# Yiming-M/CLIP-EBC

Hardware: AMD Instinct MI355X
Metric: train crops/sec clip_vit_b_16 224px @1/2/4/8 MI355X; MAE parity (higher is better)
Workload: dtype fp16; 1 GPU; clip_vit_b_16 224x224 deep-VPT(32) + DACE/DMCount train step, 16 crops/GPU, AMP fp16, NWPU anchors (BASELINE configs[2]); global_batch=16, seq_len=229, parallelism=dp1

## Files before the change

### clip-ebc_amd/csrc/attention.hip

```cpp
#include <algorithm>
#include <cstdlib>
#include <string>

#include "ebc_common.h"
#include "kernels.h"
#include "mfma.h"
#include "touch.h"

using namespace ebc;

#ifndef EBC_ATTN_STAMP
#define EBC_ATTN_STAMP(phase) ((void)0)
#endif

namespace {

constexpr int HD = 64;
constexpr int LP = 256;
constexpr int NKT = LP / 16;
constexpr float LOG2E = 1.4426950408889634f;
__device__ __forceinline__ int attn_block() { return xcd_remap(blockIdx.x, (int)gridDim.x); }

template <class E> struct AttnCfg {
    using T = typename E::T;
// ... 364 lines not shown
#pragma unroll
            for (int dt = 0; dt < HD / 16; ++dt) row[16 * dt + fr] = E::from(dq_acc[dt][i] * scale);
        }
    }
}

template <class E, int NWV, int LFIX>
__global__ __launch_bounds__(64 * NWV) void attn_bwd_dq_kernel(const typename E::T* __restrict__ qkv, const typename E::T* __restrict__ dout,
                                                          const typename E::T* __restrict__ out, const float* __restrict__ lse,
                                                          float* __restrict__ delta, typename E::T* __restrict__ dqkv, int B,
                                                          int L_, int H, float scale)
{
    attn_bwd_dq_body<E, NWV, LFIX>(attn_block(), qkv, dout, out, lse, delta, dqkv, B, L_, H, scale);
}

template <class E>
__device__ __forceinline__ float attn_delta_row(const typename E::T* drow, const typename E::T* orow) {
    float p[4];
#pragma unroll
    for (int fg = 0; fg < 4; ++fg) {
        float dd = 0.f;
#pragma unroll
        for (int ks = 0; ks < 2; ++ks) {
            const typename E::Frag df = load8<E>(drow + 32 * ks + 8 * fg), of = load8<E>(orow + 32 * ks + 8 * fg);
#pragma unroll
            for (int j = 0; j < 8; ++j) dd = fmaf((float)df[j], (float)of[j], dd);
        }
        p[fg] = dd;
    }
    return (p[0] + p[1]) + (p[2] + p[3]);
}

template <class E>
__device__ __forceinline__ float attn_delta_quad(const typename E::T* drow, const typename E::T* orow) {
    const typename E::Frag d0 = load8<E>(drow), d1 = load8<E>(drow + 8), o0 = load8<E>(orow), o1 = load8<E>(orow + 8);
    float acc = 0.f;
#pragma unroll
    for (int j = 0; j < 8; j += 2) {
        if constexpr (std::is_same<E, EF16>::value) {
            typedef _Float16 h2 __attribute__((ext_vector_type(2)));
            acc = __builtin_amdgcn_fdot2(h2{d0[j], d0[j + 1]}, h2{o0[j], o0[j + 1]}, acc, false);
            acc = __builtin_amdgcn_fdot2(h2{d1[j], d1[j + 1]}, h2{o1[j], o1[j + 1]}, acc, false);
        } else {
            typedef __bf16 b2 __attribute__((ext_vector_type(2)));
            acc = __builtin_amdgcn_fdot2_f32_bf16(b2{d0[j], d0[j + 1]}, b2{o0[j], o0[j + 1]}, acc, false);
            acc = __builtin_amdgcn_fdot2_f32_bf16(b2{d1[j], d1[j + 1]}, b2{o1[j], o1[j + 1]}, acc, false);
        }
    }
    acc += __builtin_amdgcn_update_dpp(0.f, acc, 0xB1, 0xF, 0xF, false);
    acc += __builtin_amdgcn_update_dpp(0.f, acc, 0x4E, 0xF, 0xF, false);
    return acc;
}

template <class E, int NWV, int LFIX>
__device__ __forceinline__ void attn_bwd_dkv_body(int bid, const typename E::T* __restrict__ qkv, const typename E::T* __restrict__ dout,
                                                  const typename E::T* __restrict__ out, const float* __restrict__ lse,
                                                  const float* __restrict__ delta, typename E::T* __restrict__ dqkv, int B,
                                                  int L_, int H, float scale)
{
    const int L = LFIX > 0 ? LFIX : L_;
    using T = typename E::T;
    using C = AttnCfg<E>;
    extern __shared__ __attribute__((aligned(16))) char smem[];
    T* Qs = reinterpret_cast<T*>(smem);
    T* Ds = reinterpret_cast<T*>(smem + C::TILE_BYTES);
    float* ls = reinterpret_cast<float*>(smem + 2 * C::TILE_BYTES);
    float* dl = ls + LP;
    constexpr int QB = 16 * NWV;
    const int nkb = (L + QB - 1) / QB;
    const int bh = bid / nkb, kb = bid % nkb;
    const int b = bh / H, h = bh % H;
    const int D3 = 3 * H * HD, D = H * HD;
    const T* base = qkv + (size_t)b * L * D3 + h * HD;
    RowFetch<E, NWV> fq, fd;
    rows_fetch<E, NWV>(fq, base, D3, L);
    rows_fetch<E, NWV>(fd, dout + (size_t)b * L * D + h * HD, D, L);
    const int lane = threadIdx.x & 63, w = threadIdx.x >> 6, fr = lane & 15, fg = lane >> 4;
    const int k0 = kb * QB + w * 16;
    const int kme = k0 + fr;
    const bool kv = kme < L;
    typename E::Frag kf[2], vf[2];
#pragma unroll
    for (int ks = 0; ks < 2; ++ks) {
        kf[ks] = gload8<E>(base + (size_t)kme * D3 + D + 32 * ks + 8 * fg, kv);
// ... 64 lines not shown
                                                           const float* __restrict__ lse, const float* __restrict__ delta,
                                                           typename E::T* __restrict__ dqkv, int B, int L_, int H, float scale)
{
    attn_bwd_dkv_body<E, NWV, LFIX>(attn_block(), qkv, dout, nullptr, lse, delta, dqkv, B, L_, H, scale);
}

struct AttnLaneOffsets {
    int row[2];
    int col[HD / 16];
    __device__ __forceinline__ AttnLaneOffsets() {
        const int l = threadIdx.x & 63, fr = l & 15, fg = l >> 4;
        const int sr = attn_swz(fr);
#pragma unroll
        for (int ks = 0; ks < 2; ++ks) row[ks] = (fr * HD + (((4 * ks + fg) ^ sr) << 3)) * 2;
        const int g = l >> 4, w = l & 15, q = w >> 2, p = w & 3, rr = 4 * g + q, sc = attn_swz(rr);
#pragma unroll
        for (int dt = 0; dt < HD / 16; ++dt) col[dt] = (rr * HD + ((((2 * dt + (p >> 1)) ^ sc) << 3) | (4 * (p & 1)))) * 2;
    }
};
template <class E>
__device__ __forceinline__ typename E::Frag rowfrag_at(const char* tile, int off, int t) {
    return __builtin_bit_cast(typename E::Frag, *reinterpret_cast<const uint4*>(tile + off + t * 16 * HD * 2));
}
template <class E>
__device__ __forceinline__ typename E::Frag colfrag_at(const char* tile, int off, int st) {
    const char* a = tile + off + st * 32 * HD * 2;
    const s16x4 lo = __builtin_amdgcn_ds_read_tr16_b64_v4i16((__attribute__((address_space(3))) s16x4*)(a));
    const s16x4 hi = __builtin_amdgcn_ds_read_tr16_b64_v4i16((__attribute__((address_space(3))) s16x4*)(a + 16 * HD * 2));
    typedef short s16x8 __attribute__((ext_vector_type(8)));
    s16x8 v = {lo[0], lo[1], lo[2], lo[3], hi[0], hi[1], hi[2], hi[3]};
    return __builtin_bit_cast(typename E::Frag, v);
}

template <class E, int LFIX>
__global__ __launch_bounds__(1024) void attn_bwd_one_kernel(const typename E::T* __restrict__ qkv, const typename E::T* __restrict__ dout,
                                                           const typename E::T* __restrict__ out, const float* __restrict__ lse,
                                                           typename E::T* __restrict__ dqkv, int B, int L_, int H, float scale,
                                                           int rows, TouchList touch)
{
    constexpr int NWV = 16;
    const int L = LFIX > 0 ? LFIX : L_;
    using T = typename E::T;
    using C = AttnCfg<E>;
    EBC_ATTN_STAMP(0);
    extern __shared__ __attribute__((aligned(16))) char smem[];
    T* Ks = reinterpret_cast<T*>(smem);
    T* Vs = reinterpret_cast<T*>(smem + C::TILE_BYTES);
    T* Qs = reinterpret_cast<T*>(smem + 2 * C::TILE_BYTES);
    T* Ds = reinterpret_cast<T*>(smem + 3 * C::TILE_BYTES);
    float* ls = reinterpret_cast<float*>(smem + 4 * C::TILE_BYTES);
    float* dl = ls + LP;
    const int bh = attn_block(), b = bh / H, h = bh % H;
    const int D3 = 3 * H * HD, D = H * HD;
    const T* base = qkv + (size_t)b * L * D3 + h * HD;
    const T* dob = dout + (size_t)b * L * D + h * HD;
    RowFetch<E, NWV> fk, fv, fq, fd;
    rows_fetch<E, NWV>(fk, base + D, D3, L);
    rows_fetch<E, NWV>(fv, base + 2 * D, D3, L);
    rows_fetch<E, NWV>(fq, base, D3, L);
    rows_fetch<E, NWV>(fd, dob, D, L);
    const int qd = threadIdx.x >> 2, qj = threadIdx.x & 3;
    float lsv = INFINITY, dlv = 0.f;
    if (qd < L) {
        if (qj == 0) lsv = lse[((size_t)b * H + h) * L + qd] * LOG2E;
        dlv = attn_delta_quad<E>(dob + (size_t)qd * D + 16 * qj, out + ((size_t)b * L + qd) * D + h * HD + 16 * qj);
    }
    rows_store<E, NWV>(Ks, fk);
    rows_store<E, NWV>(Vs, fv);
    rows_store<E, NWV>(Qs, fq);
    rows_store<E, NWV>(Ds, fd);
    static_assert(64 * NWV >= 4 * LP, "a lane quad per padded query");
    if (qj == 0) { ls[qd] = lsv; dl[qd] = dlv; }
    __syncthreads();
    EBC_ATTN_STAMP(1);

    const int lane = threadIdx.x & 63, w = threadIdx.x >> 6, fr = lane & 15, fg = lane >> 4;
    const int lim = rows > 0 && rows < L ? rows : L;
    TouchSink tsink;
    if (touch.n) touch_issue<NWV>(touch, tsink);
    if (16 * w >= lim) {
        if (touch.n) touch_wait(tsink);
        EBC_ATTN_STAMP(2);
        return;
    }
    const int nkt = (L + 15) >> 4;
    const bool ragged = (L & 15) != 0;
    const float c2 = scale * LOG2E;
    static_assert(E::BYTES == 2, "swizzled 16-bit tiles");
    const AttnLaneOffsets lo;
    const char* Kr[2] = {reinterpret_cast<const char*>(Ks) + lo.row[0], reinterpret_cast<const char*>(Ks) + lo.row[1]};
    const char* Vr[2] = {reinterpret_cast<const char*>(Vs) + lo.row[0], reinterpret_cast<const char*>(Vs) + lo.row[1]};
    const char* Qr[2] = {reinterpret_cast<const char*>(Qs) + lo.row[0], reinterpret_cast<const char*>(Qs) + lo.row[1]};
    const char* Dr[2] = {reinterpret_cast<const char*>(Ds) + lo.row[0], reinterpret_cast<const char*>(Ds) + lo.row[1]};
    const char* Kc[HD / 16];
    const char* Qc[HD / 16];
    const char* Dc[HD / 16];
#pragma unroll
    for (int dt = 0; dt < HD / 16; ++dt) {
        Kc[dt] = reinterpret_cast<const char*>(Ks) + lo.col[dt];
        Qc[dt] = reinterpret_cast<const char*>(Qs) + lo.col[dt];
        Dc[dt] = reinterpret_cast<const char*>(Ds) + lo.col[dt];
    }
    {
        const int q0 = 16 * w, qme = q0 + fr;
        typename E::Frag qf[2], df[2];
// ... 510 lines not shown
    return EBC_OK;
}
template <class E> int attn_fwd_t(const void* qkv, void* out, float* lse, int B, int L, int H, hipStream_t st,
                                  const TouchList* touch)
{
    if (attn_fwd_waves(B, L, H) == 16)
        return L == L_VPT32 ? attn_fwd_nw<E, 16, L_VPT32>(qkv, out, lse, B, L, H, st, touch)
                            : attn_fwd_nw<E, 16, 0>(qkv, out, lse, B, L, H, st, touch);
    return L == L_VPT32 ? attn_fwd_nw<E, 8, L_VPT32>(qkv, out, lse, B, L, H, st, touch)
                        : attn_fwd_nw<E, 8, 0>(qkv, out, lse, B, L, H, st, touch);
}

template <class E, int NW, int LFIX> int attn_bwd_nw(const void* qkv, const void* dout, const void* out, const float* lse,
                                                     float* delta, void* dqkv, int B, int L, int H, hipStream_t st)
{
    using C = AttnCfg<E>;
    const size_t lds_dq = 2 * C::TILE_BYTES, lds_kv = 2 * C::TILE_BYTES + 2 * LP * sizeof(float);
    if (!ensure_lds<attn_bwd_dq_kernel<E, NW, LFIX>>((int)lds_dq, st) || !ensure_lds<attn_bwd_dkv_kernel<E, NW, LFIX>>((int)lds_kv, st))
        return EBC_E_LAUNCH;
    const int grid = B * H * ((L + 16 * NW - 1) / (16 * NW));
    int pi = probe_on() ? probe_start(EBC_PROBE_ATTN_BWD_DQ, 0, 0, 0, 0, B, L, H, st) : -1;
    hipLaunchKernelGGL((attn_bwd_dq_kernel<E, NW, LFIX>), dim3(grid), dim3(64 * NW), lds_dq, st, (const typename E::T*)qkv,
                       (const typename E::T*)dout, (const typename E::T*)out, lse, delta, (typename E::T*)dqkv, B, L, H,
                       0.125f);
    probe_stop(pi, st);
    EBC_CHECK_LAUNCH();
    pi = probe_on() ? probe_start(EBC_PROBE_ATTN_BWD_DKV, 0, 0, 0, 0, B, L, H, st) : -1;
    hipLaunchKernelGGL((attn_bwd_dkv_kernel<E, NW, LFIX>), dim3(grid), dim3(64 * NW), lds_kv, st, (const typename E::T*)qkv,
                       (const typename E::T*)dout, lse, delta, (typename E::T*)dqkv, B, L, H, 0.125f);
    probe_stop(pi, st);
    EBC_CHECK_LAUNCH();
    return EBC_OK;
}
template <class E, int LFIX> int attn_bwd_one(const void* qkv, const void* dout, const void* out, const float* lse,
                                              void* dqkv, int B, int L, int H, hipStream_t st, int rows, const TouchList* touch)
{
    using C = AttnCfg<E>;
    const size_t lds = 4 * C::TILE_BYTES + 2 * LP * sizeof(float);
    if (!ensure_lds<attn_bwd_one_kernel<E, LFIX>>((int)lds, st)) return EBC_E_LAUNCH;
    const TouchList t = touch && g_touch_mode == 1 ? *touch : TouchList{};
    const int pi = probe_on() ? probe_start(EBC_PROBE_ATTN_BWD_DQ, 1, 0, 0, 0, B, L, H, st) : -1;
    hipLaunchKernelGGL((attn_bwd_one_kernel<E, LFIX>), dim3(B * H), dim3(1024), lds, st, (const typename E::T*)qkv,
                       (const typename E::T*)dout, (const typename E::T*)out, lse, (typename E::T*)dqkv, B, L, H, 0.125f,
                       rows, t);
    probe_stop(pi, st);
    EBC_CHECK_LAUNCH();
    return EBC_OK;
}


template <class E> int attn_bwd_t(const void* qkv, const void* dout, const void* out, const float* lse, float* delta,
                                  void* dqkv, int B, int L, int H, hipStream_t st, int rows, const TouchList* touch)
{
    if constexpr (E::BYTES == 2) {
        return L == L_VPT32 ? attn_bwd_one<E, L_VPT32>(qkv, dout, out, lse, dqkv, B, L, H, st, rows, touch)
                            : attn_bwd_one<E, 0>(qkv, dout, out, lse, dqkv, B, L, H, st, rows, touch);
    }
    if (attn_waves(L) == 16)
        return L == L_VPT32 ? attn_bwd_nw<E, 16, L_VPT32>(qkv, dout, out, lse, delta, dqkv, B, L, H, st)
                            : attn_bwd_nw<E, 16, 0>(qkv, dout, out, lse, delta, dqkv, B, L, H, st);
    return attn_bwd_nw<E, 8, 0>(qkv, dout, out, lse, delta, dqkv, B, L, H, st);
}

}

namespace ebc {
bool touch_enabled() { return g_touch_mode == 1; }
}

extern "C" int ebc_set_weight_touch(int mode)
{
    if (mode < 0 || mode > 1) return EBC_E_ARG;
    g_touch_mode = mode;
    return EBC_OK;
}

namespace ebc {
// ... 6 lines not shown
            case EBC_F32: return attn_fwd_long<EF32>(qkv, out, lse, B, L, H, st);
            case EBC_F16: return attn_fwd_long<EF16>(qkv, out, lse, B, L, H, st);
            case EBC_BF16: return attn_fwd_long<EBF16>(qkv, out, lse, B, L, H, st);
        }
        return EBC_E_ARG;
    }
    switch (dtype) {
        case EBC_F32: return attn_fwd_t<EF32>(qkv, out, lse, B, L, H, st, nullptr);
        case EBC_F16: return attn_fwd_t<EF16>(qkv, out, lse, B, L, H, st, touch);
        case EBC_BF16: return attn_fwd_t<EBF16>(qkv, out, lse, B, L, H, st, touch);
    }
    return EBC_E_ARG;
}
int attention_bwd(int dtype, const void* qkv, const void* dout, const void* out, const float* lse, float* delta,
                  void* dqkv, int B, int L, int H, hipStream_t st, int rows, const TouchList* touch)
{
    if (L <= 0 || L > L_MAX || B <= 0 || H <= 0 || rows < 0) return EBC_E_UNSUPPORTED;
    if (L > LP) {
        if (!delta || !lse) return EBC_E_ARG;
        switch (dtype) {
            case EBC_F32: return attn_bwd_long<EF32>(qkv, dout, out, lse, delta, dqkv, B, L, H, st);
            case EBC_F16: return attn_bwd_long<EF16>(qkv, dout, out, lse, delta, dqkv, B, L, H, st);
            case EBC_BF16: return attn_bwd_long<EBF16>(qkv, dout, out, lse, delta, dqkv, B, L, H, st);
        }
        return EBC_E_ARG;
    }
    switch (dtype) {
        case EBC_F32: return attn_bwd_t<EF32>(qkv, dout, out, lse, delta, dqkv, B, L, H, st, rows, nullptr);
        case EBC_F16: return attn_bwd_t<EF16>(qkv, dout, out, lse, delta, dqkv, B, L, H, st, rows, touch);
        case EBC_BF16: return attn_bwd_t<EBF16>(qkv, dout, out, lse, delta, dqkv, B, L, H, st, rows, touch);
    }
    return EBC_E_ARG;
}
}
```

### clip-ebc_amd/csrc/kernels.h

```cpp
#pragma once
#include <hip/hip_runtime.h>
#include <stddef.h>

namespace ebc {
struct TouchList {
    const void* ptr[8];
    size_t bytes[8];
    int n;
    void add(const void* p, size_t b) { if (p && b >= 128 && n < 8) { ptr[n] = p; bytes[n] = b; ++n; } }
};
bool touch_enabled();
bool probe_on();
int probe_start(int kind, int epi, int bm, int bn, int mode, int m, int n, int k, hipStream_t st);
void probe_stop(int idx, hipStream_t st);
int gemm_nt(int dtype, int epi, int out_f32, const void* A, const void* B, void* C, const float* bias,
            const float* resid, void* aux, int M, int N, int K, hipStream_t st, void* ws = nullptr,
            size_t ws_bytes = 0, int a_rpg = 0, int a_gstride = 0, int a_goff = 0);
struct GemmLn {
    void* xh = nullptr;
    float* rpart = nullptr;
    const float* lnp = nullptr;
    int lnparts = 0;
    const float* lnw = nullptr;
    float* mean = nullptr;
// ... 30 lines not shown
int layernorm_fwd(int dtype, const float* x, int rpg, int gstride, int goff, const float* gamma, const float* beta,
                  void* out, float* outf, float* mean, float* rstd, int M, int D, hipStream_t st);
int layernorm_bwd_fill(int dtype, const float* dy, const float* x, int rpg, int gstride, int goff, const float* mean,
                       const float* rstd, const float* gamma, float* dx_out, void* dx_out_t, int M, int D, hipStream_t st,
                       const TouchList* touch = nullptr);
int layernorm_bwd(int dtype, int dy_f32, const void* dy, const float* x, int rpg, int gstride, int goff,
                  const float* mean, const float* rstd, const float* gamma, const float* dx_in, float* dx_out,
                  void* dx_out_t, int M, int D, hipStream_t st);
int im2col(int dtype, const float* x, void* out, int B, int H, int W, int P, hipStream_t st);
int embed_tokens(const float* patch, const float* cls, const float* pos, const float* gamma, const float* beta,
                 const float* vpt, long vpt_bstride, float* X, int B, int L, int G, int NVPT, int D, hipStream_t st);
int layernorm_fwd_vpt(int dtype, float* X, const float* vpt, long vpt_bstride, int L, int NVPT, const float* gamma,
                      const float* beta, void* out, float* mean, float* rstd, int M, int D, hipStream_t st);
int layernorm_bwd_vpt(int dtype, const void* dy, const float* x, const float* mean, const float* rstd,
                      const float* gamma, const float* dx_in, float* dx_out, void* dx_out_t, int M, int D, float* vpt_rows,
                      int L, int NVPT, hipStream_t st);
int vpt_sum(const float* rows, float* const* dst, int layers, int B, int NVPT, int D, hipStream_t st);
int insert_vpt(float* X, const float* vpt, long vpt_bstride, int B, int L, int NVPT, int D, hipStream_t st);
int vpt_grad(int dtype, float* dX, void* dXt, float* dvpt, int B, int L, int NVPT, int D, int per_batch, int accumulate,
             hipStream_t st);
int head_fwd(int dtype_z, const void* Z, const float* text, const float* logit_scale, const float* anchors,
             float* logits, float* expo, int P, int HW, int NB, int embed, hipStream_t st);
size_t head_bwd_ws_bytes(int P, int embed);
int head_bwd(int dtype_z, int dtype_dz, const void* Z, const float* text, const float* logit_scale, const float* anchors,
             const float* dlogits, const float* dexp, const float* gscale, void* dZ, float* dbias, float* dscale,
             int P, int HW, int NB, int embed, void* ws, size_t wsb, hipStream_t st);
int attn_delta(int dtype, const void* dO, const void* O, float* delta, int B, int L, int H, hipStream_t st);
int cast_f32(int dtype, const float* in, void* out, size_t n, hipStream_t st);
int attention_fwd(int dtype, const void* qkv, void* out, float* lse, int B, int L, int H, hipStream_t st,
                  const TouchList* touch = nullptr);
int attention_bwd(int dtype, const void* qkv, const void* dout, const void* out, const float* lse, float* delta,
                  void* dqkv, int B, int L, int H, hipStream_t st, int rows = 0,
                  const TouchList* touch = nullptr);
int layernorm_bwd_rows(int dtype, const void* dy, const float* x, int rpg, int gstride, int goff, const float* mean,
                       const float* rstd, const float* gamma, const float* dx_in, float* dx_out, int M, int D,
                       hipStream_t st);
}

#define EBC_TRY(x)                  \
    do {                            \
        int _rc = (x);              \
        if (_rc != 0) return _rc;   \
    } while (0)
```

### clip-ebc_amd/csrc/vit.hip

```cpp
#include <vector>

#include <algorithm>

#include "ebc_common.h"
#include "kernels.h"


namespace {

constexpr int WIDTH = 768, HEADS = 12, MLP = 3072, QKVW = 3 * WIDTH;

inline size_t align_up(size_t x) { return (x + 255) & ~(size_t)255; }

struct Carver {
    char* base; size_t off = 0; bool dry;
    Carver(void* b, bool d) : base((char*)b), dry(d) {}
    template <class P> P* take(size_t bytes) {
        P* p = dry ? nullptr : reinterpret_cast<P*>(base + off);
        off += align_up(bytes);
        return p;
    }
};

struct LayerSave {
// ... 217 lines not shown
    };
    for (int l = 0; l < layers; ++l) EBC_TRY(block(l, 0, B, st));
    EBC_TRY(ebc::layernorm_fwd(EBC_F32, lay.X[layers], G, L, 1 + NV, w->ln_post_g, w->ln_post_b, feat, nullptr,
                               lay.mpost, lay.rpost, B * G, WIDTH, st));
    return EBC_OK;
}

extern "C" int ebc_vit_backward(const EbcVitWeights* w, int B, int H, int W, int dtype, void* ws, size_t ws_bytes,
                                const float* dfeat, float* const* dvpt, long vpt_bstride, int flags, ebc_stream_t stream)
{
    if (!check_weights(w) || !ws || !dfeat || B <= 0 || H < w->patch || W < w->patch || H % w->patch || W % w->patch)
        return EBC_E_ARG;
    hipStream_t st = (hipStream_t)stream;
    const int P = w->patch;
    const int NV = w->num_vpt, G = (H / P) * (W / P), L = 1 + NV + G, layers = w->layers;
    const int M = B * L;
    Layout lay = carve(ws, B, L, G, 3 * P * P, layers, dtype, 1);
    if (lay.bytes > ws_bytes) return EBC_E_ARG;
    const int per_batch = vpt_bstride != 0;

    float* dX = lay.dXa;
    float* dXo = lay.dXb;
    if (lay.gws && hipMemsetAsync(lay.gws, 0, std::min<size_t>(lay.gws_bytes, 16 * 1024), st) != hipSuccess)
        return EBC_E_LAUNCH;
    auto gemm = [&](int epi, const void* A, const void* Bm, void* C, void* aux, int m, int n, int k) {
        return ebc::gemm_nt(dtype, epi, 0, A, Bm, C, nullptr, nullptr, aux, m, n, k, st, lay.gws, lay.gws_bytes);
    };
    bool fold_b = dtype != EBC_F32 && lay.bpart && !(flags & EBC_VIT_BWD_NO_LN_FOLD) &&
                  ebc::gemm_ln_bwd_fold_pays(dtype, M, WIDTH, MLP);
    for (int l = 0; l < layers && fold_b; ++l) {
        const EbcVitLayer& p = w->layer[l];
        fold_b = p.wt_fc_ln && p.s_fc_ln && p.b_fc_ln;
    }
    const size_t es = dtype == EBC_F32 ? 4 : 2;
    auto touch_bwd = [&](int l) {
        ebc::TouchList t{};
        if (l < layers) t.add(w->layer[l].wt_qkv, (size_t)WIDTH * QKVW * es);
        if (l > 0) {
            const EbcVitLayer& q = w->layer[l - 1];
            t.add(q.wt_proj, (size_t)MLP * WIDTH * es);
            t.add(fold_b ? q.wt_fc_ln : q.wt_fc, (size_t)WIDTH * MLP * es);
            t.add(q.wt_out, (size_t)WIDTH * WIDTH * es);
        }
        return t;
    };
    const ebc::TouchList tl_top = touch_bwd(layers);
    EBC_TRY(ebc::layernorm_bwd_fill(dtype, dfeat, lay.X[layers], G, L, 1 + NV, lay.mpost, lay.rpost, w->ln_post_g, dX,
                                    lay.dXt, B * G, WIDTH, st, dtype != EBC_F32 ? &tl_top : nullptr));
    for (int l = layers - 1; l >= 0; --l) {
        const EbcVitLayer& p = w->layer[l];
        LayerSave& s = lay.s[l];
        const ebc::TouchList tl = touch_bwd(l);
        if (fold_b) {
            ebc::GemmLn gb;
            gb.bpart = lay.bpart; gb.lnb_s = p.s_fc_ln; gb.lnb_c = p.b_fc_ln;
            EBC_TRY(ebc::gemm_nt_ln(dtype, EBC_EPI_GELU_BWD, 0, lay.dXt, p.wt_proj, lay.dA, nullptr, nullptr, s.A, M, MLP,
                                    WIDTH, st, lay.gws, lay.gws_bytes, gb));
            ebc::GemmLn lb;
            lb.xh = lay.dXt; lb.lnx = s.X1; lb.lnp = lay.bpart; lb.lnparts = lay.parts_gelu; lb.mean = s.m2; lb.rstd = s.r2;
            EBC_TRY(ebc::gemm_nt_ln(dtype, ebc::GEMM_EPI_LN_BWD, 1, lay.dA, p.wt_fc_ln, dXo, nullptr, dX, nullptr, M, WIDTH,
                                    MLP, st, lay.gws, lay.gws_bytes, lb));
        } else {
            EBC_TRY(gemm(EBC_EPI_GELU_BWD, lay.dXt, p.wt_proj, lay.dA, s.A, M, MLP, WIDTH));
            EBC_TRY(gemm(EBC_EPI_STORE, lay.dA, p.wt_fc, lay.dH, nullptr, M, WIDTH, MLP));
            EBC_TRY(ebc::layernorm_bwd(dtype, 0, lay.dH, s.X1, 0, 0, 0, s.m2, s.r2, p.ln2_g, dX, dXo, lay.dXt, M, WIDTH, st));
        }
        { float* t = dX; dX = dXo; dXo = t; }
        EBC_TRY(gemm(EBC_EPI_STORE, lay.dXt, p.wt_out, lay.dO, nullptr, M, WIDTH, WIDTH));
        if (l == 0 && NV > 0 && dvpt && dvpt[0] && !(flags & EBC_VIT_BWD_FULL_LAYER0)) {
            EBC_TRY(ebc::attention_bwd(dtype, s.QKV, lay.dO, s.O, s.lse, lay.delta, lay.dQKV, B, L, HEADS, st, 1 + NV, &tl));
            EBC_TRY(ebc::gemm_nt(dtype, EBC_EPI_STORE, 0, lay.dQKV, p.wt_qkv, lay.dH, nullptr, nullptr, nullptr, B * NV,
                                 WIDTH, QKVW, st, lay.gws, lay.gws_bytes, NV, L, 1));
            float* rows = per_batch ? dvpt[0] : lay.vpt_rows;
            EBC_TRY(ebc::layernorm_bwd_rows(dtype, lay.dH, lay.X[0], NV, L, 1, s.m1, s.r1, p.ln1_g, dX, rows, B * NV,
                                            WIDTH, st));
            break;
        }
        EBC_TRY(ebc::attention_bwd(dtype, s.QKV, lay.dO, s.O, s.lse, lay.delta, lay.dQKV, B, L, HEADS, st, 0, &tl));
        EBC_TRY(gemm(EBC_EPI_STORE, lay.dQKV, p.wt_qkv, lay.dH, nullptr, M, WIDTH, QKVW));
        if (NV > 0 && dvpt && dvpt[l]) {
            float* rows = per_batch ? dvpt[l] : lay.vpt_rows + (size_t)l * B * NV * WIDTH;
            EBC_TRY(ebc::layernorm_bwd_vpt(dtype, lay.dH, lay.X[l], s.m1, s.r1, p.ln1_g, dX, dXo, lay.dXt, M, WIDTH,
                                           rows, L, NV, st));
        } else {
            EBC_TRY(ebc::layernorm_bwd(dtype, 0, lay.dH, lay.X[l], 0, 0, 0, s.m1, s.r1, p.ln1_g, dX, dXo, lay.dXt, M, WIDTH, st));
        }
        { float* t = dX; dX = dXo; dXo = t; }
    }
    if (NV > 0 && dvpt && !per_batch) EBC_TRY(ebc::vpt_sum(lay.vpt_rows, dvpt, layers, B, NV, WIDTH, st));
    return EBC_OK;
}

extern "C" int ebc_layernorm_fwd(int dtype, const float* x, int rows_per_group, int group_stride, int group_offset,
                                 const float* gamma, const float* beta, void* out, float* out_f32, float* mean,
                                 float* rstd, int M, int D, ebc_stream_t stream)
{
    return ebc::layernorm_fwd(dtype, x, rows_per_group, group_stride, group_offset, gamma, beta, out, out_f32, mean,
                              rstd, M, D, (hipStream_t)stream);
}
extern "C" int ebc_layernorm_bwd(int dtype, int dy_f32, const void* dy, const float* x, int rows_per_group,
                                 int group_stride, int group_offset, const float* mean, const float* rstd,
                                 const float* gamma, const float* dx_in, float* dx_out, void* dx_out_t, int M, int D,
                                 ebc_stream_t stream)
{
    return ebc::layernorm_bwd(dtype, dy_f32, dy, x, rows_per_group, group_stride, group_offset, mean, rstd, gamma,
                              dx_in, dx_out, dx_out_t, M, D, (hipStream_t)stream);
}
extern "C" int ebc_attention_fwd(int dtype, const void* qkv, void* out, float* lse, int B, int L, int H, ebc_stream_t stream)
{
    return ebc::attention_fwd(dtype, qkv, out, lse, B, L, H, (hipStream_t)stream);
}
extern "C" int ebc_attention_bwd(int dtype, const void* qkv, const void* dout, const void* out, const float* lse,
                                 float* delta_ws, void* dqkv, int B, int L, int H, ebc_stream_t stream)
{
    return ebc::attention_bwd(dtype, qkv, dout, out, lse, delta_ws, dqkv, B, L, H, (hipStream_t)stream);
}
extern "C" int ebc_head_fwd(int dtype_z, const void* Z, const float* text, const float* logit_scale, const float* anchors,
                            float* logits, float* expo, int P, int HW, int NB, int embed, ebc_stream_t stream)
{
    return ebc::head_fwd(dtype_z, Z, text, logit_scale, anchors, logits, expo, P, HW, NB, embed, (hipStream_t)stream);
}
extern "C" size_t ebc_head_bwd_workspace_bytes(int P, int embed)
{
    return ebc::head_bwd_ws_bytes(P, embed);
}
extern "C" int ebc_head_bwd(int dtype_z, int dtype_dz, const void* Z, const float* text, const float* logit_scale,
                            const float* anchors, const float* dlogits, const float* dexp, const float* gscale, void* dZ,
                            float* dbias, float* dscale, int P, int HW, int NB, int embed, void* workspace,
                            size_t workspace_bytes, ebc_stream_t stream)
{
    return ebc::head_bwd(dtype_z, dtype_dz, Z, text, logit_scale, anchors, dlogits, dexp, gscale, dZ, dbias, dscale, P, HW,
                         NB, embed, workspace, workspace_bytes, (hipStream_t)stream);
}
extern "C" int ebc_im2col(int dtype, const float* x, void* out, int B, int H, int W, int patch, ebc_stream_t stream)
{
    if (!x || !out || B <= 0 || patch <= 0 || H < patch || W < patch) return EBC_E_ARG;
    return ebc::im2col(dtype, x, out, B, H, W, patch, (hipStream_t)stream);
}
extern "C" int ebc_cast_f32(int dtype, const float* in, void* out, size_t n, ebc_stream_t stream)
{
    return ebc::cast_f32(dtype, in, out, n, (hipStream_t)stream);
}
```

### clip-ebc_amd/ebc_amd/_lib.py

```python
from __future__ import annotations

import ctypes
import os
from typing import Optional

import torch

PKG_ROOT = os.path.dirname(os.path.dirname(os.path.abspath(__file__)))
LIB_PATH = os.environ.get("EBC_LIB_PATH") or os.path.join(PKG_ROOT, "lib", "libebc_hip.so")

EBC_F32, EBC_F16, EBC_BF16 = 0, 1, 2
EBC_COUNT_DMCOUNT, EBC_COUNT_MAE, EBC_COUNT_MSE, EBC_COUNT_OT_ONLY = 0, 1, 2, 3
_ERR = {-1: "EBC_E_ARG", -2: "EBC_E_LAUNCH", -3: "EBC_E_UNSUPPORTED"}

_lib: Optional[ctypes.CDLL] = None

_P = ctypes.c_void_p
_I = ctypes.c_int
_F = ctypes.c_float
_Z = ctypes.c_size_t
_D = ctypes.c_double
_L = ctypes.c_long


# ... 23 lines not shown

class EbcAdamTensor(ctypes.Structure):
    _fields_ = [("param", ctypes.c_void_p), ("grad", ctypes.c_void_p), ("exp_avg", ctypes.c_void_p),
                ("exp_avg_sq", ctypes.c_void_p), ("numel", ctypes.c_long)]


SIGNATURES = {
    "ebc_version": (_I, []),
    "ebc_dace_workspace_bytes": (_Z, [_I, _I, _I, _I]),
    "ebc_scale2": (_I, [_P, _P, _P, _L, _P, _P, _L, _P]),
    "ebc_dace_loss_h": (_I, [_P, _P, _P, _I, _P, _P, _P, _P, _P, _I, _I, _I, _I, _I, _I, _F, _F, _F, _F, _I, _F, _I,
                             _P, _P, _P, _P, _P, _P, _P, _Z, _P]),
    "ebc_dace_loss": (_I, [_P, _P, _P, _I, _P, _P, _P, _P, _P, _I, _I, _I, _I, _I, _I, _F, _F, _F, _F, _I, _F, _I,
                           _P, _P, _P, _P, _P, _P, _P, _Z, _P]),
    "ebc_sinkhorn_workspace_bytes": (_Z, [_I, _I]),
    "ebc_sinkhorn": (_I, [_P, _P, _P, _I, _I, _F, _I, _F, _I, _I, _P, _P, _P, _P, _P, _P, _P, _P, _Z, _P]),
    "ebc_gemm": (_I, [_I, _I, _I, _P, _P, _P, _P, _P, _P, _I, _I, _I, _P]),
    "ebc_gemm_workspace_bytes": (_Z, [_I, _I, _I, _I]),
    "ebc_gemm_tile_config": (_I, [_I, _I, _I, _I, _P]),
    "ebc_conv_tile_config": (_I, [_I, _I, _I, _I, _I, _P]),
    "ebc_gemm_ws": (_I, [_I, _I, _I, _P, _P, _P, _P, _P, _P, _I, _I, _I, _P, _Z, _P]),
    "ebc_gemm_wgrad_workspace_bytes": (_Z, [_I, _I, _I, _I]),
    "ebc_gemm_wgrad": (_I, [_I, _P, _P, _P, _I, _I, _I, _P, _Z, _P]),
    "ebc_transpose": (_I, [_I, _P, _P, _I, _I, _L, _P]),
    "ebc_vit_workspace_bytes": (_Z, [_I, _I, _I, _I, _I, _I, _I]),
    "ebc_vit_workspace_bytes_p": (_Z, [_I, _I, _I, _I, _I, _I, _I, _I]),
    "ebc_vit_forward": (_I, [_P, _P, _I, _I, _I, _P, ctypes.c_long, _I, _I, _P, _Z, _P, _P]),
    "ebc_vit_backward": (_I, [_P, _I, _I, _I, _I, _P, _Z, _P, _P, ctypes.c_long, _I, _P]),
    "ebc_set_weight_touch": (_I, [_I]),
    "ebc_layernorm_fwd": (_I, [_I, _P, _I, _I, _I, _P, _P, _P, _P, _P, _P, _I, _I, _P]),
    "ebc_layernorm_bwd": (_I, [_I, _I, _P, _P, _I, _I, _I, _P, _P, _P, _P, _P, _P, _I, _I, _P]),
    "ebc_attention_fwd": (_I, [_I, _P, _P, _P, _I, _I, _I, _P]),
    "ebc_attention_bwd": (_I, [_I, _P, _P, _P, _P, _P, _P, _I, _I, _I, _P]),
    "ebc_head_fwd": (_I, [_I, _P, _P, _P, _P, _P, _P, _I, _I, _I, _I, _P]),
    "ebc_head_bwd": (_I, [_I, _I, _P, _P, _P, _P, _P, _P, _P, _P, _P, _P, _I, _I, _I, _I, _P, _Z, _P]),
    "ebc_head_bwd_workspace_bytes": (_Z, [_I, _I]),
    "ebc_cast_f32": (_I, [_I, _P, _P, _Z, _P]),
    "ebc_im2col": (_I, [_I, _P, _P, _I, _I, _I, _I, _P]),
    "ebc_tile_gather": (_I, [_P, _P, _I, _I, _I, _I, _I, _I, _I, _I, _I, _P]),
    "ebc_tile_assemble": (_I, [_P, _P, _I, _I, _I, _I, _I, _I, _I, _I, _P]),
    "ebc_dec_geometry": (_I, [_I, _I, _I, _I, _I, _P]),
    "ebc_dec_workspace_bytes": (_Z, [_I, _I, _I, _I, _I, _I]),
    "ebc_dec_upsample_pad": (_I, [_I, _P, _P, _I, _I, _I, _I, _I, _P]),
    "ebc_conv3x3_fwd": (_I, [_I, _P, _P, _P, _P, _P, _P, _P, _Z, _I, _I, _I, _I, _I, _P]),
    "ebc_conv3x3_wgrad": (_I, [_I, _P, _P, _P, _P, _Z, _I, _I, _I, _I, _I, _P]),
    "ebc_bn_finalize": (_I, [_P, _D, _F, _F, _P, _P, _P, _P, _P, _P, _P, _P, _P, _I, _P]),
    "ebc_conv3x3_fwd_bn": (_I, [_I, _P, _P, _P, _P, _Z, _I, _I, _I, _I, _I, _F, _F, _P, _P, _P, _P, _P, _P, _P, _P,
                                _P, _P, _P]),
    "ebc_bn_relu_pad": (_I, [_I, _P, _P, _P, _P, _I, _I, _I, _I, _P]),
    "ebc_bn_add_relu": (_I, [_I, _P, _P, _P, _P, _I, _P, _I, _I, _I, _I, _P]),
    "ebc_bn_bwd_reduce": (_I, [_I, _P, _P, _P, _P, _P, _P, _P, _P, _P, _Z, _L, _I, _P]),
    "ebc_bn_bwd_finalize": (_I, [_P, _D, _P, _P, _P, _P, _P, _I, _P]),
    "ebc_bn_bwd_apply": (_I, [_I, _P, _P, _P, _P, _P, _P, _P, _P, _P, _P, _I, _I, _I, _I, _P]),
    "ebc_dec_transpose3": (_I, [_I, _P, _P, _I, _I, _I, _I, _P]),
    "ebc_dec_prep_weights": (_I, [_I, _P, _P, _P, _I, _I, _P]),
    "ebc_dec_upsample_bwd": (_I, [_I, _P, _P, _I, _I, _I, _I, _I, _P]),
    "ebc_dec_upsample": (_I, [_I, _P, _P, _I, _I, _I, _I, _I, _P]),
    "ebc_bn_stats": (_I, [_I, _P, _P, _P, _Z, _L, _I, _P]),
    "ebc_bn_stats_finalize": (_I, [_I, _P, _P, _Z, _L, _I, _F, _F, _P, _P, _P, _P, _P, _P, _P, _P, _P, _P, _P]),
    "ebc_bn_bwd_reduce_finalize": (_I, [_I, _P, _P, _P, _P, _P, _P, _P, _P, _P, _P, _P, _P, _Z, _L, _I, _P]),
    "ebc_bn_relu": (_I, [_I, _P, _P, _P, _P, _L, _I, _P]),
    "ebc_bn_bwd_apply_flat": (_I, [_I, _P, _P, _P, _P, _P, _P, _P, _P, _P, _P, _L, _I, _P]),
    "ebc_bn_relu_avgpool": (_I, [_I, _P, _P, _P, _P, _I, _I, _I, _I, _P]),
    "ebc_avgpool2": (_I, [_I, _I, _P, _P, _I, _I, _I, _I, _P]),
    "ebc_avgpool2_bwd": (_I, [_I, _I, _P, _P, _I, _I, _I, _I, _P]),
    "ebc_bn_add_relu_flat": (_I, [_I, _P, _P, _P, _P, _P, _P, _P, _L, _I, _P]),
# ... 67 lines not shown
```

### include/ebc_hip.h

```cpp
#ifndef EBC_HIP_H
#define EBC_HIP_H

#include <stddef.h>
#include <stdint.h>

#ifdef __cplusplus
extern "C" {
#endif

typedef void* ebc_stream_t;

enum { EBC_F32 = 0, EBC_F16 = 1, EBC_BF16 = 2 };
enum { EBC_OK = 0, EBC_E_ARG = -1, EBC_E_LAUNCH = -2, EBC_E_UNSUPPORTED = -3 };
enum { EBC_COUNT_DMCOUNT = 0, EBC_COUNT_MAE = 1, EBC_COUNT_MSE = 2, EBC_COUNT_OT_ONLY = 3 };

int ebc_version(void);

size_t ebc_dace_workspace_bytes(int B, int total_points, int size, int reduction);
int ebc_scale2(const float* s, const float* a, float* a_out, long na, const float* b, float* b_out, long nb,
               ebc_stream_t stream);
int ebc_dace_loss(const float* pred_class, const float* pred_density, const float* target_density,
                  int target_is_reduced, const float* points, const int* offsets, const int* order,
                  const float* bins_lo, const float* bins_hi, int B, int N, int size, int reduction,
                  int count_mode, int norm_cood, float weight_count_loss, float weight_ot, float weight_tv,
// ... 24 lines not shown
                const float* bias, const float* resid, void* aux, int M, int N, int K,
                void* workspace, size_t workspace_bytes, ebc_stream_t stream);
size_t ebc_gemm_wgrad_workspace_bytes(int dtype, int M, int N, int K);
int ebc_gemm_wgrad(int dtype, const void* A, const void* B, float* C, int M, int N, int K,
                   void* workspace, size_t workspace_bytes, ebc_stream_t stream);
int ebc_transpose(int dtype, const void* in, void* out, int R, int C, long ld_out, ebc_stream_t stream);

typedef struct {
    const void* w_qkv;  const float* b_qkv;
    const void* w_out;  const float* b_out;
    const void* w_fc;   const float* b_fc;
    const void* w_proj; const float* b_proj;
    const float* ln1_g; const float* ln1_b; const float* ln2_g; const float* ln2_b;
    const void* wt_qkv; const void* wt_out; const void* wt_fc; const void* wt_proj;
    const void* w_qkv_ln; const float* b_qkv_ln; const float* s_qkv_ln;
    const void* w_fc_ln;  const float* b_fc_ln;  const float* s_fc_ln;
    const void* wt_qkv_ln; const void* wt_fc_ln;
} EbcVitLayer;

typedef struct {
    int layers, width, heads, patch, num_vpt;
    const void* w_patch;
    const float* cls;
    const float* pos;
    const float* ln_pre_g; const float* ln_pre_b; const float* ln_post_g; const float* ln_post_b;
    const EbcVitLayer* layer;
} EbcVitWeights;

size_t ebc_vit_workspace_bytes(int B, int H, int W, int layers, int num_vpt, int dtype, int training);
size_t ebc_vit_workspace_bytes_p(int B, int H, int W, int patch, int layers, int num_vpt, int dtype, int training);
int ebc_vit_forward(const EbcVitWeights* w, const float* image, int B, int H, int W,
                    const float* const* vpt, long vpt_bstride, int dtype, int training,
                    void* workspace, size_t workspace_bytes, float* feat, ebc_stream_t stream);
enum { EBC_VIT_BWD_FULL_LAYER0 = 1, EBC_VIT_BWD_NO_LN_FOLD = 2 };
int ebc_vit_backward(const EbcVitWeights* w, int B, int H, int W, int dtype, void* workspace,
                     size_t workspace_bytes, const float* dfeat, float* const* dvpt, long vpt_bstride, int flags,
                     ebc_stream_t stream);

int ebc_layernorm_fwd(int dtype, const float* x, int rows_per_group, int group_stride, int group_offset,
                      const float* gamma, const float* beta, void* out, float* out_f32, float* mean,
                      float* rstd, int M, int D, ebc_stream_t stream);
int ebc_layernorm_bwd(int dtype, int dy_f32, const void* dy, const float* x, int rows_per_group,
                      int group_stride, int group_offset, const float* mean, const float* rstd,
                      const float* gamma, const float* dx_in, float* dx_out, void* dx_out_t, int M, int D,
                      ebc_stream_t stream);
int ebc_attention_fwd(int dtype, const void* qkv, void* out, float* lse, int B, int L, int H, ebc_stream_t stream);
int ebc_attention_bwd(int dtype, const void* qkv, const void* dout, const void* out, const float* lse,
                      float* delta_ws, void* dqkv, int B, int L, int H, ebc_stream_t stream);
int ebc_head_fwd(int dtype_z, const void* Z, const float* text, const float* logit_scale, const float* anchors,
                 float* logits, float* expo, int P, int HW, int NB, int embed, ebc_stream_t stream);
size_t ebc_head_bwd_workspace_bytes(int P, int embed);
int ebc_head_bwd(int dtype_z, int dtype_dz, const void* Z, const float* text, const float* logit_scale,
                 const float* anchors, const float* dlogits, const float* dexp, const float* gscale, void* dZ,
                 float* dbias, float* dscale, int P, int HW, int NB, int embed, void* workspace, size_t workspace_bytes,
                 ebc_stream_t stream);
int ebc_cast_f32(int dtype, const float* in, void* out, size_t n, ebc_stream_t stream);
int ebc_im2col(int dtype, const float* x, void* out, int B, int H, int W, int patch, ebc_stream_t stream);

int ebc_tile_gather(const float* image, float* tiles, int C, int H, int W, int wh, int ww, int sh, int sw,
                    int tile_begin, int tile_count, ebc_stream_t stream);
int ebc_tile_assemble(const float* preds, float* out, int Cp, int H, int W, int wh, int ww, int sh, int sw,
                      int reduction, ebc_stream_t stream);

#define EBC_AUG_MAX_BLUR 31
typedef struct {
    int64_t src_off, out_off, tmp_off;
    int64_t noise_off;
    int32_t src_h, src_w, top, left, crop_h, crop_w, out_h, out_w;
    int32_t flip, jitter_ops;
    float brightness, contrast, saturation;
    int32_t blur, noise;
    float saltiness, spiciness;
    uint32_t seed;
    int32_t normalize;
    float hue;
} EbcCropDesc;
typedef struct {
    float mean[3], std[3];
    int32_t blur_k;
    float sigma_x, sigma_y;
} EbcAugConst;
// ... 95 lines not shown
```

Baseline: 3825 crops/s.

## Fuse out-projection backward GEMM into single-block attention backward kernel

```diff
diff --git a/clip-ebc_amd/csrc/attention.hip b/clip-ebc_amd/csrc/attention.hip
--- a/clip-ebc_amd/csrc/attention.hip
+++ b/clip-ebc_amd/csrc/attention.hip
@@ -420,8 +420,8 @@
 }
 
 template <class E>
-__device__ __forceinline__ float attn_delta_quad(const typename E::T* drow, const typename E::T* orow) {
-    const typename E::Frag d0 = load8<E>(drow), d1 = load8<E>(drow + 8), o0 = load8<E>(orow), o1 = load8<E>(orow + 8);
+__device__ __forceinline__ float attn_delta_quad_f(const typename E::Frag& d0, const typename E::Frag& d1,
+                                                   const typename E::Frag& o0, const typename E::Frag& o1) {
     float acc = 0.f;
 #pragma unroll
     for (int j = 0; j < 8; j += 2) {
@@ -438,6 +438,11 @@
     acc += __builtin_amdgcn_update_dpp(0.f, acc, 0xB1, 0xF, 0xF, false);
     acc += __builtin_amdgcn_update_dpp(0.f, acc, 0x4E, 0xF, 0xF, false);
     return acc;
+}
+template <class E>
+__device__ __forceinline__ float attn_delta_quad(const typename E::T* drow, const typename E::T* orow) {
+    const typename E::Frag d0 = load8<E>(drow), d1 = load8<E>(drow + 8), o0 = load8<E>(orow), o1 = load8<E>(orow + 8);
+    return attn_delta_quad_f<E>(d0, d1, o0, o1);
 }
 
 template <class E, int NWV, int LFIX>
@@ -568,8 +573,11 @@
     return __builtin_bit_cast(typename E::Frag, v);
 }
 
-template <class E, int LFIX>
+constexpr int PROJ_MAX_H = 12;
+__device__ __forceinline__ int proj_swz(int r) { return (0x1320 >> (((r >> 2) & 3) * 4)) & 3; }
+template <class E, int LFIX, bool PROJ = false>
 __global__ __launch_bounds__(1024) void attn_bwd_one_kernel(const typename E::T* __restrict__ qkv, const typename E::T* __restrict__ dout,
+                                                           const typename E::T* __restrict__ wt,
                                                            const typename E::T* __restrict__ out, const float* __restrict__ lse,
                                                            typename E::T* __restrict__ dqkv, int B, int L_, int H, float scale,
                                                            int rows, TouchList touch)
@@ -590,23 +598,112 @@
     const int D3 = 3 * H * HD, D = H * HD;
     const T* base = qkv + (size_t)b * L * D3 + h * HD;
     const T* dob = dout + (size_t)b * L * D + h * HD;
+    const int pl = threadIdx.x & 63, pw = threadIdx.x >> 6, pfr = pl & 15, pfg = pl >> 4;
+    const int nks = D / 32;
+    constexpr int MAXU = (8 * PROJ_MAX_H + NWV - 1) / NWV, XC = PROJ ? 6 : 1;
+    const int prow = 16 * pw + pfr;
+    const bool plive = 16 * pw < L;
+    const int xr = 16 * pw + (pl >> 2);
+    const T* xrow = dout + ((size_t)b * L + (xr < L ? xr : 0)) * D + 8 * (pl & 3);
+    typename E::Frag x0[XC], x1[XC];
+    auto xload = [&](typename E::Frag (&xf)[XC], int kc) {
+#pragma unroll
+        for (int j = 0; j < XC; ++j) xf[j] = load8<E>(xrow + 32 * min(kc + j, nks - 1));
+    };
+    if constexpr (PROJ) {
+        const int nu = 4 * nks, upw = (nu + NWV - 1) / NWV;
+        const T* wsrc = wt + ((size_t)h * HD + (pl >> 2)) * D + 8 * ((pl & 3) ^ proj_swz(pl >> 2));
+#pragma unroll
+        for (int i = 0; i < MAXU; ++i) {
+            const int u = min(pw * upw + i, nu - 1), nb = u / nks, kk = u - nb * nks;
+            __builtin_amdgcn_global_load_lds((const __attribute__((address_space(1))) void*)(wsrc + (size_t)16 * nb * D + 32 * kk),
+                                             EBC_LDS(smem + kk * 4096 + nb * 1024), 16, 0, 0);
+        }
+        asm volatile("" ::: "memory");
+        xload(x0, 0);
+        asm volatile("s_waitcnt vmcnt(0)" ::: "memory");
+        __syncthreads();
+        EBC_ATTN_STAMP(18);
+    }
     RowFetch<E, NWV> fk, fv, fq, fd;
-    rows_fetch<E, NWV>(fk, base + D, D3, L);
-    rows_fetch<E, NWV>(fv, base + 2 * D, D3, L);
-    rows_fetch<E, NWV>(fq, base, D3, L);
-    rows_fetch<E, NWV>(fd, dob, D, L);
     const int qd = threadIdx.x >> 2, qj = threadIdx.x & 3;
     float lsv = INFINITY, dlv = 0.f;
-    if (qd < L) {
-        if (qj == 0) lsv = lse[((size_t)b * H + h) * L + qd] * LOG2E;
-        dlv = attn_delta_quad<E>(dob + (size_t)qd * D + 16 * qj, out + ((size_t)b * L + qd) * D + h * HD + 16 * qj);
+    const T* orow = out + ((size_t)b * L + qd) * D + h * HD + 16 * qj;
+    typename E::Frag o0{}, o1{};
+    auto fetch_operands = [&]() {
+        rows_fetch<E, NWV>(fk, base + D, D3, L);
+        rows_fetch<E, NWV>(fv, base + 2 * D, D3, L);
+        rows_fetch<E, NWV>(fq, base, D3, L);
+        if constexpr (!PROJ) rows_fetch<E, NWV>(fd, dob, D, L);
+        if (qd < L) {
+            if (qj == 0) {
+                lsv = lse[((size_t)b * H + h) * L + qd];
+                if constexpr (!PROJ) lsv *= LOG2E;
+            }
+            if constexpr (!PROJ) dlv = attn_delta_quad<E>(dob + (size_t)qd * D + 16 * qj, orow);
+        }
+    };
+    if constexpr (!PROJ) fetch_operands();
+    static_assert(64 * NWV >= 4 * LP, "a lane quad per padded query");
+    if constexpr (PROJ) {
+        f32x4 pacc[HD / 16];
+#pragma unroll
+        for (int nb = 0; nb < HD / 16; ++nb) pacc[nb] = f32x4{0.f, 0.f, 0.f, 0.f};
+        if (plive) {
+            const char* wfr = smem + pfr * 64 + ((pfg ^ proj_swz(pfr)) << 4);
+            const int xsrc = 4 * (4 * pfr + pfg);
+            auto pstep = [&](const typename E::Frag (&xf)[XC], int kc) {
+#pragma unroll
+                for (int j = 0; j < XC; ++j) {
+                    if (kc + j < nks) {
+                        const char* wp = wfr + (kc + j) * 4096;
+                        const uint4 raw = __builtin_bit_cast(uint4, xf[j]);
+                        const uint4 xp = make_uint4(__builtin_amdgcn_ds_bpermute(xsrc, raw.x), __builtin_amdgcn_ds_bpermute(xsrc, raw.y),
+                                                    __builtin_amdgcn_ds_bpermute(xsrc, raw.z), __builtin_amdgcn_ds_bpermute(xsrc, raw.w));
+                        const typename E::Frag xb = __builtin_bit_cast(typename E::Frag, xp);
+#pragma unroll
+                        for (int nb = 0; nb < HD / 16; ++nb)
+                            pacc[nb] = mma(__builtin_bit_cast(typename E::Frag, *reinterpret_cast<const uint4*>(wp + nb * 1024)),
+                                           xb, pacc[nb]);
+                    }
+                }
+            };
+            for (int kc = 0; kc < nks; kc += 2 * XC) {
+                const bool last = kc + 2 * XC >= nks;
+                xload(x1, kc + XC);
+                if (last) fetch_operands();
+                pstep(x0, kc);
+                if (!last) xload(x0, kc + 2 * XC);
+                pstep(x1, kc + XC);
+            }
+        } else {
+            fetch_operands();
+        }
+        if (qd < L) { o0 = load8<E>(orow); o1 = load8<E>(orow + 8); }
+        __syncthreads();
+        EBC_ATTN_STAMP(19);
+        typedef T t4 __attribute__((ext_vector_type(4)));
+#pragma unroll
+        for (int nb = 0; nb < HD / 16; ++nb) {
+            t4 v = t4{E::from(pacc[nb][0]), E::from(pacc[nb][1]), E::from(pacc[nb][2]), E::from(pacc[nb][3])};
+            if (prow >= L) v = t4{E::from(0.f), E::from(0.f), E::from(0.f), E::from(0.f)};
+            *reinterpret_cast<t4*>(Ds + attn_off<E>(prow, 16 * nb + 4 * pfg)) = v;
+        }
     }
     rows_store<E, NWV>(Ks, fk);
     rows_store<E, NWV>(Vs, fv);
     rows_store<E, NWV>(Qs, fq);
-    rows_store<E, NWV>(Ds, fd);
-    static_assert(64 * NWV >= 4 * LP, "a lane quad per padded query");
-    if (qj == 0) { ls[qd] = lsv; dl[qd] = dlv; }
+    if constexpr (!PROJ) rows_store<E, NWV>(Ds, fd);
+    if constexpr (PROJ) {
+        asm volatile("" : "+v"(lsv));
+        if (qj == 0) ls[qd] = lsv * LOG2E;
+        __syncthreads();
+        if (qd < L)
+            dlv = attn_delta_quad_f<E>(load8<E>(Ds + attn_off<E>(qd, 16 * qj)), load8<E>(Ds + attn_off<E>(qd, 16 * qj + 8)), o0, o1);
+        if (qj == 0) dl[qd] = dlv;
+    } else {
+        if (qj == 0) { ls[qd] = lsv; dl[qd] = dlv; }
+    }
     __syncthreads();
     EBC_ATTN_STAMP(1);
 
@@ -1183,17 +1280,19 @@
     EBC_CHECK_LAUNCH();
     return EBC_OK;
 }
-template <class E, int LFIX> int attn_bwd_one(const void* qkv, const void* dout, const void* out, const float* lse,
-                                              void* dqkv, int B, int L, int H, hipStream_t st, int rows, const TouchList* touch)
+template <class E, int LFIX, bool PROJ = false>
+int attn_bwd_one(const void* qkv, const void* dout, const void* out, const float* lse, void* dqkv, int B, int L, int H,
+                 hipStream_t st, int rows, const TouchList* touch, const void* wt = nullptr)
 {
     using C = AttnCfg<E>;
     const size_t lds = 4 * C::TILE_BYTES + 2 * LP * sizeof(float);
-    if (!ensure_lds<attn_bwd_one_kernel<E, LFIX>>((int)lds, st)) return EBC_E_LAUNCH;
+    if (PROJ && (!wt || H > PROJ_MAX_H)) return EBC_E_UNSUPPORTED;
+    if (!ensure_lds<attn_bwd_one_kernel<E, LFIX, PROJ>>((int)lds, st)) return EBC_E_LAUNCH;
     const TouchList t = touch && g_touch_mode == 1 ? *touch : TouchList{};
     const int pi = probe_on() ? probe_start(EBC_PROBE_ATTN_BWD_DQ, 1, 0, 0, 0, B, L, H, st) : -1;
-    hipLaunchKernelGGL((attn_bwd_one_kernel<E, LFIX>), dim3(B * H), dim3(1024), lds, st, (const typename E::T*)qkv,
-                       (const typename E::T*)dout, (const typename E::T*)out, lse, (typename E::T*)dqkv, B, L, H, 0.125f,
-                       rows, t);
+    hipLaunchKernelGGL((attn_bwd_one_kernel<E, LFIX, PROJ>), dim3(B * H), dim3(1024), lds, st, (const typename E::T*)qkv,
+                       (const typename E::T*)dout, (const typename E::T*)wt, (const typename E::T*)out, lse,
+                       (typename E::T*)dqkv, B, L, H, 0.125f, rows, t);
     probe_stop(pi, st);
     EBC_CHECK_LAUNCH();
     return EBC_OK;
@@ -1266,4 +1365,19 @@
     }
     return EBC_E_ARG;
 }
-}
+bool attention_bwd_proj_ok(int dtype, int L, int H)
+{
+    return (dtype == EBC_F16 || dtype == EBC_BF16) && L > 0 && L <= LP && H > 0 && H <= PROJ_MAX_H;
+}
+int attention_bwd_proj(int dtype, const void* qkv, const void* dx, const void* wt_out, const void* out, const float* lse,
+                       void* dqkv, int B, int L, int H, hipStream_t st, int rows, const TouchList* touch)
+{
+    if (B <= 0 || rows < 0 || !attention_bwd_proj_ok(dtype, L, H)) return EBC_E_UNSUPPORTED;
+    if (!qkv || !dx || !wt_out || !out || !lse || !dqkv) return EBC_E_ARG;
+    if (dtype == EBC_F16)
+        return L == L_VPT32 ? attn_bwd_one<EF16, L_VPT32, true>(qkv, dx, out, lse, dqkv, B, L, H, st, rows, touch, wt_out)
+                            : attn_bwd_one<EF16, 0, true>(qkv, dx, out, lse, dqkv, B, L, H, st, rows, touch, wt_out);
+    return L == L_VPT32 ? attn_bwd_one<EBF16, L_VPT32, true>(qkv, dx, out, lse, dqkv, B, L, H, st, rows, touch, wt_out)
+                        : attn_bwd_one<EBF16, 0, true>(qkv, dx, out, lse, dqkv, B, L, H, st, rows, touch, wt_out);
+}
+}
diff --git a/clip-ebc_amd/csrc/kernels.h b/clip-ebc_amd/csrc/kernels.h
--- a/clip-ebc_amd/csrc/kernels.h
+++ b/clip-ebc_amd/csrc/kernels.h
@@ -86,6 +86,9 @@
 int attention_bwd(int dtype, const void* qkv, const void* dout, const void* out, const float* lse, float* delta,
                   void* dqkv, int B, int L, int H, hipStream_t st, int rows = 0,
                   const TouchList* touch = nullptr);
+bool attention_bwd_proj_ok(int dtype, int L, int H);
+int attention_bwd_proj(int dtype, const void* qkv, const void* dx, const void* wt_out, const void* out, const float* lse,
+                       void* dqkv, int B, int L, int H, hipStream_t st, int rows = 0, const TouchList* touch = nullptr);
 int layernorm_bwd_rows(int dtype, const void* dy, const float* x, int rpg, int gstride, int goff, const float* mean,
                        const float* rstd, const float* gamma, const float* dx_in, float* dx_out, int M, int D,
                        hipStream_t st);
diff --git a/clip-ebc_amd/csrc/vit.hip b/clip-ebc_amd/csrc/vit.hip
--- a/clip-ebc_amd/csrc/vit.hip
+++ b/clip-ebc_amd/csrc/vit.hip
@@ -273,6 +273,7 @@
         const EbcVitLayer& p = w->layer[l];
         fold_b = p.wt_fc_ln && p.s_fc_ln && p.b_fc_ln;
     }
+    const bool do_fuse = !(flags & EBC_VIT_BWD_NO_DO_FUSE) && ebc::attention_bwd_proj_ok(dtype, L, HEADS);
     const size_t es = dtype == EBC_F32 ? 4 : 2;
     auto touch_bwd = [&](int l) {
         ebc::TouchList t{};
@@ -307,9 +308,14 @@
             EBC_TRY(ebc::layernorm_bwd(dtype, 0, lay.dH, s.X1, 0, 0, 0, s.m2, s.r2, p.ln2_g, dX, dXo, lay.dXt, M, WIDTH, st));
         }
         { float* t = dX; dX = dXo; dXo = t; }
-        EBC_TRY(gemm(EBC_EPI_STORE, lay.dXt, p.wt_out, lay.dO, nullptr, M, WIDTH, WIDTH));
+        auto attn_bwd = [&](int rows) {
+            if (do_fuse)
+                return ebc::attention_bwd_proj(dtype, s.QKV, lay.dXt, p.wt_out, s.O, s.lse, lay.dQKV, B, L, HEADS, st, rows, &tl);
+            return ebc::attention_bwd(dtype, s.QKV, lay.dO, s.O, s.lse, lay.delta, lay.dQKV, B, L, HEADS, st, rows, &tl);
+        };
+        if (!do_fuse) EBC_TRY(gemm(EBC_EPI_STORE, lay.dXt, p.wt_out, lay.dO, nullptr, M, WIDTH, WIDTH));
         if (l == 0 && NV > 0 && dvpt && dvpt[0] && !(flags & EBC_VIT_BWD_FULL_LAYER0)) {
-            EBC_TRY(ebc::attention_bwd(dtype, s.QKV, lay.dO, s.O, s.lse, lay.delta, lay.dQKV, B, L, HEADS, st, 1 + NV, &tl));
+            EBC_TRY(attn_bwd(1 + NV));
             EBC_TRY(ebc::gemm_nt(dtype, EBC_EPI_STORE, 0, lay.dQKV, p.wt_qkv, lay.dH, nullptr, nullptr, nullptr, B * NV,
                                  WIDTH, QKVW, st, lay.gws, lay.gws_bytes, NV, L, 1));
             float* rows = per_batch ? dvpt[0] : lay.vpt_rows;
@@ -317,7 +323,7 @@
                                             WIDTH, st));
             break;
         }
-        EBC_TRY(ebc::attention_bwd(dtype, s.QKV, lay.dO, s.O, s.lse, lay.delta, lay.dQKV, B, L, HEADS, st, 0, &tl));
+        EBC_TRY(attn_bwd(0));
         EBC_TRY(gemm(EBC_EPI_STORE, lay.dQKV, p.wt_qkv, lay.dH, nullptr, M, WIDTH, QKVW));
         if (NV > 0 && dvpt && dvpt[l]) {
             float* rows = per_batch ? dvpt[l] : lay.vpt_rows + (size_t)l * B * NV * WIDTH;
@@ -356,6 +362,11 @@
 {
     return ebc::attention_bwd(dtype, qkv, dout, out, lse, delta_ws, dqkv, B, L, H, (hipStream_t)stream);
 }
+extern "C" int ebc_attention_bwd_proj(int dtype, const void* qkv, const void* dx, const void* wt_out, const void* out,
+                                      const float* lse, void* dqkv, int B, int L, int H, int rows, ebc_stream_t stream)
+{
+    return ebc::attention_bwd_proj(dtype, qkv, dx, wt_out, out, lse, dqkv, B, L, H, (hipStream_t)stream, rows);
+}
 extern "C" int ebc_head_fwd(int dtype_z, const void* Z, const float* text, const float* logit_scale, const float* anchors,
                             float* logits, float* expo, int P, int HW, int NB, int embed, ebc_stream_t stream)
 {
diff --git a/clip-ebc_amd/ebc_amd/_lib.py b/clip-ebc_amd/ebc_amd/_lib.py
--- a/clip-ebc_amd/ebc_amd/_lib.py
+++ b/clip-ebc_amd/ebc_amd/_lib.py
@@ -79,6 +79,7 @@
     "ebc_layernorm_bwd": (_I, [_I, _I, _P, _P, _I, _I, _I, _P, _P, _P, _P, _P, _P, _I, _I, _P]),
     "ebc_attention_fwd": (_I, [_I, _P, _P, _P, _I, _I, _I, _P]),
     "ebc_attention_bwd": (_I, [_I, _P, _P, _P, _P, _P, _P, _I, _I, _I, _P]),
+    "ebc_attention_bwd_proj": (_I, [_I, _P, _P, _P, _P, _P, _P, _I, _I, _I, _I, _P]),
     "ebc_head_fwd": (_I, [_I, _P, _P, _P, _P, _P, _P, _I, _I, _I, _I, _P]),
     "ebc_head_bwd": (_I, [_I, _I, _P, _P, _P, _P, _P, _P, _P, _P, _P, _P, _I, _I, _I, _I, _P, _Z, _P]),
     "ebc_head_bwd_workspace_bytes": (_Z, [_I, _I]),
diff --git a/include/ebc_hip.h b/include/ebc_hip.h
--- a/include/ebc_hip.h
+++ b/include/ebc_hip.h
@@ -80,7 +80,7 @@
 int ebc_vit_forward(const EbcVitWeights* w, const float* image, int B, int H, int W,
                     const float* const* vpt, long vpt_bstride, int dtype, int training,
                     void* workspace, size_t workspace_bytes, float* feat, ebc_stream_t stream);
-enum { EBC_VIT_BWD_FULL_LAYER0 = 1, EBC_VIT_BWD_NO_LN_FOLD = 2 };
+enum { EBC_VIT_BWD_FULL_LAYER0 = 1, EBC_VIT_BWD_NO_LN_FOLD = 2, EBC_VIT_BWD_NO_DO_FUSE = 4 };
 int ebc_vit_backward(const EbcVitWeights* w, int B, int H, int W, int dtype, void* workspace,
                      size_t workspace_bytes, const float* dfeat, float* const* dvpt, long vpt_bstride, int flags,
                      ebc_stream_t stream);
@@ -95,6 +95,8 @@
 int ebc_attention_fwd(int dtype, const void* qkv, void* out, float* lse, int B, int L, int H, ebc_stream_t stream);
 int ebc_attention_bwd(int dtype, const void* qkv, const void* dout, const void* out, const float* lse,
                       float* delta_ws, void* dqkv, int B, int L, int H, ebc_stream_t stream);
+int ebc_attention_bwd_proj(int dtype, const void* qkv, const void* dx, const void* wt_out, const void* out,
+                           const float* lse, void* dqkv, int B, int L, int H, int rows, ebc_stream_t stream);
 int ebc_head_fwd(int dtype_z, const void* Z, const float* text, const float* logit_scale, const float* anchors,
                  float* logits, float* expo, int P, int HW, int NB, int embed, ebc_stream_t stream);
 size_t ebc_head_bwd_workspace_bytes(int P, int embed);
```

Measured after the change: 3850 crops/s (median of 6 runs). Within noise of the previous version (+0.6%).
